# Arief-AK/OpenCL-Development-Real-time-Image-Processing

Measured on AMD Instinct MI355X. Metric: Mpixels/s (Gaussian 5x5, 4K RGBA), higher is better.
Workload: dtype u8 in/out, f32 accumulate

## Files before the change

### opencl-development-real-time-image-processing_amd/csrc/gauss_slide.hip

```cpp
#include <cmath>
#include <cstdlib>
#include <type_traits>

#include "common.hpp"
#include "kernels.hpp"
#include "slide_common.hpp"

namespace mi355 {

namespace {

constexpr uint32_t kRowStoreNowhere = 0x80000000u;
__device__ __forceinline__ void gstore_row_nt(global_ptr<uint8_t> rowp, uint32_t row_bytes, uint32_t off, u32x4 v)
{
    const auto rsrc = __builtin_amdgcn_make_buffer_rsrc((void*)rowp, (short)0, (int)row_bytes, 0x00020000);
    __builtin_amdgcn_raw_buffer_store_b128(v, rsrc, (int)off, 0, 2 );
}

constexpr uint32_t kSlideLdsForFiveWaves = 160u * 1024u / 5u - 1024u;
template <typename... KArgs, typename... Args>
hipError_t launch_slide_lds(void (*kernel)(KArgs...), const BandPlan& plan, uint32_t lds_bytes, hipStream_t stream,
                            Args... args)
{
    hipLaunchKernelGGL(kernel, dim3(plan.nblocks_a + plan.nblocks_b), dim3(kSlideWavesPerBlock * 64), lds_bytes, stream,
                       static_cast<KArgs>(args)...);
    return hipGetLastError();
}

template <int K>
struct Weights {
    float w[K];
};

__device__ __forceinline__ float ubyte_f32(uint32_t p, int c)
{
    return (float)((p >> (8 * c)) & 0xFFu);
}

__device__ __forceinline__ void cvt_pack4x4(const float (&h)[4][4] , u32x4& o)
{
    uint32_t o0, o1, o2, o3;
    asm("v_cvt_u32_f32_e32 %0, %4\n\t"
        "v_cvt_u32_f32_e32 %1, %5\n\t"
        "v_cvt_u32_f32_e32 %2, %6\n\t"
        "v_cvt_u32_f32_e32 %3, %7\n\t"
        "v_cvt_u32_f32_sdwa %0, %8 dst_sel:BYTE_1 dst_unused:UNUSED_PRESERVE src0_sel:DWORD\n\t"
        "v_cvt_u32_f32_sdwa %1, %9 dst_sel:BYTE_1 dst_unused:UNUSED_PRESERVE src0_sel:DWORD\n\t"
        "v_cvt_u32_f32_sdwa %2, %10 dst_sel:BYTE_1 dst_unused:UNUSED_PRESERVE src0_sel:DWORD\n\t"
        "v_cvt_u32_f32_sdwa %3, %11 dst_sel:BYTE_1 dst_unused:UNUSED_PRESERVE src0_sel:DWORD\n\t"
        "v_cvt_u32_f32_sdwa %0, %12 dst_sel:BYTE_2 dst_unused:UNUSED_PRESERVE src0_sel:DWORD\n\t"
        "v_cvt_u32_f32_sdwa %1, %13 dst_sel:BYTE_2 dst_unused:UNUSED_PRESERVE src0_sel:DWORD\n\t"
        "v_cvt_u32_f32_sdwa %2, %14 dst_sel:BYTE_2 dst_unused:UNUSED_PRESERVE src0_sel:DWORD\n\t"
        "v_cvt_u32_f32_sdwa %3, %15 dst_sel:BYTE_2 dst_unused:UNUSED_PRESERVE src0_sel:DWORD\n\t"
        "v_cvt_u32_f32_sdwa %0, %16 dst_sel:BYTE_3 dst_unused:UNUSED_PRESERVE src0_sel:DWORD\n\t"
        "v_cvt_u32_f32_sdwa %1, %17 dst_sel:BYTE_3 dst_unused:UNUSED_PRESERVE src0_sel:DWORD\n\t"
        "v_cvt_u32_f32_sdwa %2, %18 dst_sel:BYTE_3 dst_unused:UNUSED_PRESERVE src0_sel:DWORD\n\t"
        "v_cvt_u32_f32_sdwa %3, %19 dst_sel:BYTE_3 dst_unused:UNUSED_PRESERVE src0_sel:DWORD\n\t"
        "s_nop 1"
        : "=&v"(o0), "=&v"(o1), "=&v"(o2), "=&v"(o3)
        : "v"(h[0][0]), "v"(h[0][1]), "v"(h[0][2]), "v"(h[0][3]), "v"(h[1][0]), "v"(h[1][1]), "v"(h[1][2]),
          "v"(h[1][3]), "v"(h[2][0]), "v"(h[2][1]), "v"(h[2][2]), "v"(h[2][3]), "v"(h[3][0]), "v"(h[3][1]),
          "v"(h[3][2]), "v"(h[3][3]));
    o = u32x4{o0, o1, o2, o3};
}

__device__ __forceinline__ void cvt_pack3x4(const float (&h)[4][4] , uint32_t alpha_hi,
                                            u32x4& o)
{
    uint32_t o0, o1, o2, o3;
    asm("v_cvt_u32_f32_e32 %0, %4\n\t"
        "v_cvt_u32_f32_e32 %1, %5\n\t"
        "v_cvt_u32_f32_e32 %2, %6\n\t"
        "v_cvt_u32_f32_e32 %3, %7\n\t"
        "v_cvt_u32_f32_sdwa %0, %8 dst_sel:BYTE_1 dst_unused:UNUSED_PRESERVE src0_sel:DWORD\n\t"
        "v_cvt_u32_f32_sdwa %1, %9 dst_sel:BYTE_1 dst_unused:UNUSED_PRESERVE src0_sel:DWORD\n\t"
        "v_cvt_u32_f32_sdwa %2, %10 dst_sel:BYTE_1 dst_unused:UNUSED_PRESERVE src0_sel:DWORD\n\t"
        "v_cvt_u32_f32_sdwa %3, %11 dst_sel:BYTE_1 dst_unused:UNUSED_PRESERVE src0_sel:DWORD\n\t"
        "v_cvt_u32_f32_sdwa %0, %12 dst_sel:BYTE_2 dst_unused:UNUSED_PRESERVE src0_sel:DWORD\n\t"
        "v_cvt_u32_f32_sdwa %1, %13 dst_sel:BYTE_2 dst_unused:UNUSED_PRESERVE src0_sel:DWORD\n\t"
        "v_cvt_u32_f32_sdwa %2, %14 dst_sel:BYTE_2 dst_unused:UNUSED_PRESERVE src0_sel:DWORD\n\t"
        "v_cvt_u32_f32_sdwa %3, %15 dst_sel:BYTE_2 dst_unused:UNUSED_PRESERVE src0_sel:DWORD\n\t"
        "v_or_b32_e32 %0, %16, %0\n\t"
        "v_or_b32_e32 %1, %16, %1\n\t"
        "v_or_b32_e32 %2, %16, %2\n\t"
        "v_or_b32_e32 %3, %16, %3"
        : "=&v"(o0), "=&v"(o1), "=&v"(o2), "=&v"(o3)
        : "v"(h[0][0]), "v"(h[0][1]), "v"(h[0][2]), "v"(h[0][3]), "v"(h[1][0]), "v"(h[1][1]), "v"(h[1][2]),
          "v"(h[1][3]), "v"(h[2][0]), "v"(h[2][1]), "v"(h[2][2]), "v"(h[2][3]), "s"(alpha_hi));
    o = u32x4{o0, o1, o2, o3};
}

template <bool CLAMP>
__device__ __forceinline__ uint32_t to_u8(float a)
{
    if constexpr (CLAMP)
        a = fminf(a, 255.0f);
    return (uint32_t)a;
}

template <bool CLAMP>
__device__ __forceinline__ uint32_t pack_px(float a, float b, float c, float d)
{
    if constexpr (CLAMP) {
        a = fminf(a, 255.0f);
        b = fminf(b, 255.0f);
        c = fminf(c, 255.0f);
        d = fminf(d, 255.0f);
    }
    return (uint32_t)a | ((uint32_t)b << 8) | ((uint32_t)c << 16) | ((uint32_t)d << 24);
}

__device__ __forceinline__ void hpass5_dpp(float v0, float v1, float v2, float v3, float w0, float w1, float w2,
                                           float w3, float w4, float& o0, float& o1, float& o2, float& o3)
{
    asm volatile(
        "s_nop 1\n\t"
        "v_mul_f32_dpp %0, %6, %8 wave_shr:1 row_mask:0xf bank_mask:0xf bound_ctrl:1\n\t"
        "v_mul_f32_dpp %1, %7, %8 wave_shr:1 row_mask:0xf bank_mask:0xf bound_ctrl:1\n\t"
        "v_mul_f32_e32 %2, %8, %4\n\t"
        "v_mul_f32_e32 %3, %8, %5\n\t"
        "v_fmac_f32_dpp %0, %7, %9 wave_shr:1 row_mask:0xf bank_mask:0xf bound_ctrl:1\n\t"
        "v_fmac_f32_e32 %1, %9, %4\n\t"
        "v_fmac_f32_e32 %2, %9, %5\n\t"
        "v_fmac_f32_e32 %3, %9, %6\n\t"
        "v_fmac_f32_e32 %0, %10, %4\n\t"
        "v_fmac_f32_e32 %1, %10, %5\n\t"
        "v_fmac_f32_e32 %2, %10, %6\n\t"
        "v_fmac_f32_e32 %3, %10, %7\n\t"
        "v_fmac_f32_e32 %0, %11, %5\n\t"
        "v_fmac_f32_e32 %1, %11, %6\n\t"
        "v_fmac_f32_e32 %2, %11, %7\n\t"
        "v_fmac_f32_dpp %3, %4, %11 wave_shl:1 row_mask:0xf bank_mask:0xf bound_ctrl:1\n\t"
        "v_fmac_f32_e32 %0, %12, %6\n\t"
        "v_fmac_f32_e32 %1, %12, %7\n\t"
        "v_fmac_f32_dpp %2, %4, %12 wave_shl:1 row_mask:0xf bank_mask:0xf bound_ctrl:1\n\t"
        "v_fmac_f32_dpp %3, %5, %12 wave_shl:1 row_mask:0xf bank_mask:0xf bound_ctrl:1"
        : "=&v"(o0), "=&v"(o1), "=&v"(o2), "=&v"(o3)
        : "v"(v0), "v"(v1), "v"(v2), "v"(v3), "v"(w0), "v"(w1), "v"(w2), "v"(w3), "v"(w4));
}

struct SlideLane {
    global_ptr<const uint8_t> fin;
    global_ptr<uint8_t> fout;
    size_t row_bytes;
    SlideGeom g;
    int y0, nout, h;
    uint32_t px_off[4];
    int w;
    RaggedEdge edge;
};

template <bool NA0>
__device__ __forceinline__ bool alpha_row_differs(const u32x4& p, uint32_t nA)
{
    uint32_t t;
    if constexpr (NA0)
        t = (p.x & p.y) & (p.z & p.w);
    else
        t = ((p.x ^ nA) & (p.y ^ nA)) & ((p.z ^ nA) & (p.w ^ nA));
    return __builtin_amdgcn_ballot_w64(t < 0xFF000000u) != 0;
}

constexpr int kBandDone = 0;
constexpr int kBandAbortUniform = 1;
constexpr int kBandAbort = 2;
constexpr int kBandAbortUniformFirst = 3;

template <typename F, int... I>
__device__ __forceinline__ void static_rows_impl(F&& f, std::integer_sequence<int, I...>)
{
    (f(std::integral_constant<int, I>{}), ...);
}
template <int N, typename F>
__device__ __forceinline__ void static_rows(F&& f)
{
    static_rows_impl(f, std::make_integer_sequence<int, N>{});
}


template <int R, bool CLAMP, int NCH, bool RAGGED, bool UP, int AMODE, bool LOCKSTEP>
__device__ __forceinline__ int gauss_slide_band(const SlideLane& L, const float (&wv)[2 * R + 1], uint32_t alpha_hi,
                                                const uint32_t* __restrict__ alpha_tab, u32x4 (&q3)[2 * R + 1],
                                                bool preloaded)
{
    constexpr int K = 2 * R + 1;
    static_assert((NCH == 4) == (AMODE == 0), "AMODE 1 / 2 belong to the 3-channel pass");
    uint32_t in_off = L.g.in_off, out_off = L.g.out_off;
    [[maybe_unused]] const uint32_t out_voff = L.g.stores ? out_off : kRowStoreNowhere;
    const BandWalk W = band_walk(UP, L.y0, L.nout, R, L.h);
    uint32_t cur_nA = 0u;
    int run = 0;
    int code = kBandDone;
    const ptrdiff_t step_bytes = UP ? -(ptrdiff_t)L.row_bytes : (ptrdiff_t)L.row_bytes;
    const int y_lo = max(L.y0 - R, 0), y_hi = min(L.y0 + L.nout - 1 + R, L.h - 1);
    int y_in = W.y_first;
    auto in_p = L.fin + (size_t)clampi(y_in, y_lo, y_hi) * L.row_bytes;
    auto out_p = L.fout + (size_t)out_row(W, 0) * L.row_bytes;
    auto next_in_row = [&]() {
        const int y_next = y_in + W.y_step;
        in_p += (min(y_in, y_next) >= y_lo && max(y_in, y_next) <= y_hi) ? step_bytes : (ptrdiff_t)0;
        y_in = y_next;
    };
    auto load_row = [&]() -> u32x4 {
        const auto rowp = in_p;
        next_in_row();
        if constexpr (R <= 2)
            lane_offset_here(in_off);
        if constexpr (RAGGED) {
            if (L.w < 4) {
                u32x4 r;
#pragma unroll
                for (int j = 0; j < 4; j++)
                    r[j] = gload<uint32_t>(rowp + L.px_off[j]);
                return r;
            }
            return gload_a4<u32x4>(rowp + in_off);
        } else {
            return gload<u32x4>(rowp + in_off);
        }
    };

    constexpr int PF = (K < 3) ? K : 3;
    u32x4 q_own[K];
    u32x4 (&q)[K] = (AMODE == 0) ? q_own : q3;
    if (AMODE != 2 || !preloaded) {
#pragma unroll
        for (int u = 0; u < PF; u++)
            q[u] = load_row();
    } else {
#pragma unroll
        for (int u = 0; u < PF; u++)
            next_in_row();
    }
    if constexpr (AMODE == 1) {
        if (alpha_row_differs<true>(q[0], 0u)) {
            const uint32_t a_row = ((uint32_t)__builtin_amdgcn_readfirstlane((int)q[0].x) >> 24) & 0xFFu;
            return alpha_row_differs<false>(q[0], (a_row ^ 0xFFu) << 24) ? kBandAbort : kBandAbortUniformFirst;
        }
    }

    constexpr bool kRing = R <= 3;
    static_assert(kRing || !UP, "the accumulator form walks down only");
    float rows[K][4 * NCH] = {};

    auto do_row = [&](auto slot, auto outputs) __attribute__((always_inline)) {
        constexpr int u = decltype(slot)::value;
        constexpr bool OUT = decltype(outputs)::value;
        {
            u32x4 p_copy = q[u];
            u32x4& p = *((PF < K) ? &q[u] : &p_copy);
            if constexpr (LOCKSTEP) {
                __builtin_amdgcn_s_barrier();
            }
            if constexpr (PF < K)
                q[(u + PF) % K] = load_row();
            if (L.g.edge_strip) {
                if constexpr (!RAGGED) {
                    if (L.g.left_of_image)
                        p = u32x4{p.x, p.x, p.x, p.x};
                    if (L.g.right_of_image)
                        p = u32x4{p.w, p.w, p.w, p.w};
                } else if (L.w >= 4) {
                    if (L.g.left_of_image)
                        p = u32x4{p.x, p.x, p.x, p.x};
                    ragged_shift_clamp(p, L.edge);
                }
            }
            if constexpr (AMODE == 1) {
                if (alpha_row_differs<true>(p, 0u) && code == kBandDone) {
                    const uint32_t a_row = ((uint32_t)__builtin_amdgcn_readfirstlane((int)p.x) >> 24) & 0xFFu;
                    code = alpha_row_differs<false>(p, (a_row ^ 0xFFu) << 24) ? kBandAbort : kBandAbortUniform;
                }
            }
            if constexpr (AMODE == 2) {
                if (alpha_row_differs<false>(p, cur_nA)) {
                    const uint32_t a_new = ((uint32_t)__builtin_amdgcn_readfirstlane((int)p.x) >> 24) & 0xFFu;
                    const uint32_t nA = (a_new ^ 0xFFu) << 24;
                    if (alpha_row_differs<false>(p, nA))
                        code = kBandAbort;
                    cur_nA = nA;
                    alpha_hi = __builtin_amdgcn_readfirstlane(alpha_tab[a_new]);
                    run = 0;
                }
                run++;
            }
            if constexpr (kRing) {
#pragma unroll
                for (int px = 0; px < 4; px++)
#pragma unroll
                    for (int c = 0; c < NCH; c++)
                        rows[u][px * NCH + c] = ubyte_f32(p[px], c);
            } else {
#pragma unroll
                for (int px = 0; px < 4; px++) {
                    float f[NCH];
#pragma unroll
                    for (int c = 0; c < NCH; c++)
                        f[c] = ubyte_f32(p[px], c);
#pragma unroll
                    for (int j = 0; j < K; j++) {
                        const int sl = (u - j + K) % K;
#pragma unroll
                        for (int c = 0; c < NCH; c++)
                            rows[sl][px * NCH + c] =
                                (j == 0) ? wv[0] * f[c] : __builtin_fmaf(wv[j], f[c], rows[sl][px * NCH + c]);
                    }
                }
            }
            if constexpr (PF == K)
                q[u] = load_row();
            if constexpr (OUT) {
                if constexpr (AMODE == 2) {
                    if (run < K)
                        code = kBandAbort;
                }
                auto vsum = [&](int e) -> float {
                    if constexpr (!kRing)
                        return rows[(u + 1) % K][e];
                    float a = wv[0] * rows[UP ? u : (u + 1) % K][e];
#pragma unroll
                    for (int j = 1; j < K; j++)
                        a = __builtin_fmaf(wv[j], rows[UP ? (u - j + K) % K : (u + 1 + j) % K][e], a);
                    return a;
                };
                u32x4 o;
                if constexpr (R == 2) {
                    float hres[4][4];
#pragma unroll
                    for (int c = 0; c < NCH; c++)
                        hpass5_dpp(vsum(0 * NCH + c), vsum(1 * NCH + c), vsum(2 * NCH + c), vsum(3 * NCH + c), wv[0],
                                   wv[1], wv[2], wv[3], wv[4], hres[c][0], hres[c][1], hres[c][2], hres[c][3]);
                    if constexpr (CLAMP) {
#pragma unroll
                        for (int px = 0; px < 4; px++)
                            o[px] = (NCH == 4) ? pack_px<true>(hres[0][px], hres[1][px], hres[2][px], hres[3][px])
                                               : (pack_px<true>(hres[0][px], hres[1][px], hres[2][px], 0.0f) | alpha_hi);
                    } else if constexpr (NCH == 4) {
                        cvt_pack4x4(hres, o);
                    } else {
                        cvt_pack3x4(hres, alpha_hi, o);
                    }
                } else {
                    float v[4 * NCH];
#pragma unroll
                    for (int e = 0; e < 4 * NCH; e++)
                        v[e] = vsum(e);
#pragma unroll
                    for (int px = 0; px < 4; px++) {
                        float r4[4] = {0.0f, 0.0f, 0.0f, 0.0f};
#pragma unroll
                        for (int c = 0; c < NCH; c++) {
                            float sum = 0.0f;
#pragma unroll
                            for (int t = 0; t < K; t++) {
                                const int s = px - R + t;
                                float src;
                                if (s < 0)
                                    src = dpp_left(v[(4 + s) * NCH + c]);
                                else if (s > 3)
                                    src = dpp_right(v[(s - 4) * NCH + c]);
                                else
                                    src = v[s * NCH + c];
                                sum = (t == 0) ? wv[0] * src : __builtin_fmaf(wv[t], src, sum);
                            }
                            r4[c] = sum;
                        }
                        o[px] = pack_px<CLAMP>(r4[0], r4[1], r4[2], r4[3]);
                        if constexpr (NCH == 3)
                            o[px] |= alpha_hi;
                    }
                }
                const auto rowp = out_p;
                out_p += step_bytes;
                if constexpr (!RAGGED) {
                    gstore_row_nt(rowp, (uint32_t)L.row_bytes, out_voff, o);
                } else if (L.g.stores) {
                    if constexpr (R <= 2)
                        lane_offset_here(out_off);
                    if constexpr (RAGGED) {
                        if (L.g.edge_strip && L.g.x_lane + 3 >= L.w) {
#pragma unroll
                            for (int j = 0; j < 4; j++)
                                if (L.g.x_lane + j < L.w)
                                    gstore_a4<uint32_t>(rowp + out_off + 4 * j, o[j]);
                        } else {
                            gstore_a4<u32x4>(rowp + out_off, o);
                        }
                    } else {
                        gstore_nt<u32x4>(rowp + out_off, o);
                    }
                }
            }
        }
    };
    static_rows<2 * R>([&](auto v) __attribute__((always_inline)) { do_row(v, std::false_type{}); });
    const int ntrips = L.nout / K, rem = L.nout - ntrips * K;
    auto trip = [&]() __attribute__((always_inline)) {
        static_rows<K>([&](auto v) __attribute__((always_inline)) {
            do_row(std::integral_constant<int, (2 * R + decltype(v)::value) % K>{}, std::true_type{});
        });
    };
    constexpr int kPeeled = RAGGED ? 0 : 1;
    if (ntrips >= kPeeled) {
        if constexpr (kPeeled)
            trip();
        for (int t = kPeeled; t < ntrips && code == kBandDone; t++)
            trip();
    }
    auto rem_rows = [&](auto self, auto v) __attribute__((always_inline)) {
        constexpr int V = decltype(v)::value;
        if constexpr (V < K - 1) {
            if (V < rem) {
                do_row(std::integral_constant<int, (2 * R + V) % K>{}, std::true_type{});
                self(self, std::integral_constant<int, V + 1>{});
            }
        }
    };
    if (code == kBandDone)
        rem_rows(rem_rows, std::integral_constant<int, 0>{});
    return code;
}

template <int R, bool CLAMP, bool RAGGED, int MODE, bool LOCKSTEP>
__global__ __launch_bounds__(kSlideWavesPerBlock * 64, (R == 3 && MODE == 3) ? 3 : 1) void gauss_slide_kernel(
    const uint8_t* __restrict__ in, uint8_t* __restrict__ out, int w, int h, int nstrips, int lanes_out,
    BandPlan plan, Weights<2 * R + 1> wts, uint32_t alpha_hi, const uint32_t* __restrict__ alpha_tab,
    uint32_t* __restrict__ flags)
{
    constexpr int K = 2 * R + 1;
    const int lane = threadIdx.x & 63;
    SlideItem it;
    if (!slide_item(plan, nstrips, h, &it))
        return;
    if constexpr (MODE == 4) {
        if (flags[it.work] == 0)
            return;
    }
    SlideLane L;
    L.g = slide_geom<4>(it.strip, lanes_out, lane, w, 16u, 16u);
    L.y0 = it.y0;
    L.nout = it.nout;
    L.h = h;
    L.w = w;
    L.row_bytes = (size_t)w * 4;
    L.fin = uniform_ptr(in + it.frame * L.row_bytes * h);
    L.fout = uniform_ptr(out + it.frame * L.row_bytes * h);
    L.edge = RaggedEdge{false, false, false, false};
    if constexpr (RAGGED) {
        if (w >= 4)
            L.g.in_off = ragged_edge_setup(L.g.q_lane, L.g.q_load, w, &L.edge);
    }
#pragma unroll
    for (int j = 0; j < 4; j++)
        L.px_off[j] = (uint32_t)clampi(L.g.x_lane + j, 0, w - 1) * 4u;

    float wv[K];
#pragma unroll
    for (int j = 0; j < K; j++) {
        wv[j] = wts.w[j];
        asm volatile("" : "+v"(wv[j]));
    }

    const bool up = (it.band & 1) != 0;
    u32x4 q3[K];
    auto run = [&](auto amode, bool preloaded) -> int {
        constexpr int AMODE = decltype(amode)::value;
        constexpr int NCH = AMODE == 0 ? 4 : 3;
        if constexpr (R <= 3) {
            if (up)
                return gauss_slide_band<R, CLAMP, NCH, RAGGED, true, AMODE, LOCKSTEP>(L, wv, alpha_hi, alpha_tab, q3, preloaded);
        }
        return gauss_slide_band<R, CLAMP, NCH, RAGGED, false, AMODE, LOCKSTEP>(L, wv, alpha_hi, alpha_tab, q3, preloaded);
    };
    auto three_channels = [&]() -> int {
        int code = run(std::integral_constant<int, 1>{}, false);
        if (code == kBandAbortUniform || code == kBandAbortUniformFirst)
            code = run(std::integral_constant<int, 2>{}, code == kBandAbortUniformFirst);
        return code;
    };
    if constexpr (MODE == 0) {
        if (three_channels() != kBandDone)
            run(std::integral_constant<int, 0>{}, false);
    } else if constexpr (MODE == 3) {
        const int code = three_channels();
        if (lane == 0)
            flags[it.work] = code == kBandDone ? 0u : 1u;
    } else {
        run(std::integral_constant<int, 0>{}, false);
    }
}

template <int R>
bool slide_plan(int w, int h, int nframes, bool ragged, StripPlan* sp, BandPlan* plan)
{
    constexpr int K = 2 * R + 1;
    *sp = make_strip_plan(w);
    if (K == 5) {
        const bool big = (size_t)sp->nstrips * ((h + 23) / 24) * nframes >= 2800;
        const int rows = (big && !ragged) ? 15 : 24;
        return make_band_plan(h, sp->nstrips, nframes, 4, rows, rows, rows, 0.0, 12, plan);
    }
    return (K == 3)   ? make_band_plan(h, sp->nstrips, nframes, 5, 12, 12, 12, 0.0, 6, plan)
                      : make_band_plan(h, sp->nstrips, nframes, 3, 96, 270, 40, 0.1, 4 * R + 4, plan);
}

template <int R>
hipError_t launch_r(hipStream_t stream, const uint8_t* d_in, uint8_t* d_out, int w, int h, int nframes,
                    const GaussCoef& coef, uint32_t* d_flags)
{
    constexpr int K = 2 * R + 1;
    constexpr bool kSplit = R >= 3;
    StripPlan sp;
    BandPlan plan;
    const bool ragged = rows_ragged(w, d_in, 16, d_out, 16) || (size_t)w * 4 > kRowStoreNowhere;
    if (!slide_plan<R>(w, h, nframes, ragged, &sp, &plan) || (kSplit && !d_flags))
        return hipErrorInvalidValue;
    const int nstrips = sp.nstrips, lanes_out = sp.lanes_out;
    Weights<K> wts;
    for (int j = 0; j < K; j++)
        wts.w[j] = coef.h_w1d[j];
    double wsum = 0.0;
    for (int j = 0; j < K; j++)
        wsum += (double)coef.h_w1d[j];
    if (!coef.d_alpha_tab)
        return hipErrorInvalidValue;
    const uint32_t alpha_hi = coef.h_alpha_tab[255];
    const uint32_t* alpha_tab = coef.d_alpha_tab;
    const bool lockstep =
        R <= 2 && !ragged && nstrips % kSlideWavesPerBlock == 0 && plan.nwork_b == 0 && plan.nwork_a >= 8192u;
    const uint32_t lds_bytes = (R == 1 && !ragged) ? kSlideLdsForFiveWaves : 0u;
    auto launch = [&](auto kernel) {
        return launch_slide_lds(kernel, plan, lds_bytes, stream, d_in, d_out, w, h, nstrips, lanes_out, plan, wts, alpha_hi,
                                alpha_tab, d_flags);
    };
    return dispatch_bool(gauss_upper_clamp(wsum), [&](auto CL) {
        return dispatch_bool(ragged, [&](auto RG) {
            if constexpr (kSplit) {
                const hipError_t e = launch(gauss_slide_kernel<R, CL.value, RG.value, 3, false>);
                return e != hipSuccess ? e : launch(gauss_slide_kernel<R, CL.value, RG.value, 4, false>);
            } else if constexpr (RG.value) {
                return launch(gauss_slide_kernel<R, CL.value, true, 0, false>);
            } else {
                return dispatch_bool(
                    lockstep, [&](auto LS) { return launch(gauss_slide_kernel<R, CL.value, false, 0, LS.value>); });
            }
        });
    });
}

}

bool gauss_slide_supported(const uint8_t* d_in, const uint8_t* d_out, int w, int h, int k)
{
    (void)h;
    (void)w;
    if (k != 3 && k != 5 && k != 7 && k != 9)
        return false;
    return aligned_to(d_in, 4) && aligned_to(d_out, 4);
}

size_t gauss_slide_flag_items(int w, int h, int nframes, int k)
{
    StripPlan sp;
    BandPlan plan;
    const hipError_t e = dispatch_int(k, std::integer_sequence<int, 7, 9>{}, [&](auto K) {
        return slide_plan<K.value / 2>(w, h, nframes, false, &sp, &plan) ? hipSuccess : hipErrorInvalidValue;
    });
    return e == hipSuccess ? (size_t)plan.nwork_a + plan.nwork_b : 0;
}

hipError_t launch_gauss_slide(hipStream_t stream, const uint8_t* d_in, uint8_t* d_out, int w, int h,
                              int nframes, const GaussCoef& coef, uint32_t* d_flags)
{
    return dispatch_int(coef.k, std::integer_sequence<int, 3, 5, 7, 9>{}, [&](auto K) {
        return launch_r<K.value / 2>(stream, d_in, d_out, w, h, nframes, coef, d_flags);
    });
}

}
```

### opencl-development-real-time-image-processing_amd/csrc/slide_common.hpp

```cpp
#pragma once
#include <cstdint>
#include <cstdlib>

#include "common.hpp"

namespace mi355 {

constexpr int kSlideLanesOutMax = 62;
constexpr int kSlideWavesPerBlock = 4;

struct BandPlan {
    int rows_a, nbands_a, rows_b, nbands_b, y_split;
    uint32_t nwork_a, nwork_b, nblocks_a, nblocks_b;
};

struct StripPlan {
    int quads, nstrips, lanes_out;
};

inline StripPlan make_strip_plan(int w, int lanes_pref = 0)
{
    StripPlan s;
    s.quads = (w + 3) / 4;
    s.nstrips = (s.quads + kSlideLanesOutMax - 1) / kSlideLanesOutMax;
    s.lanes_out = (s.quads + s.nstrips - 1) / s.nstrips;
    if (lanes_pref > 0 && lanes_pref <= kSlideLanesOutMax && s.nstrips > 1) {
        s.lanes_out = lanes_pref;
        s.nstrips = (s.quads + lanes_pref - 1) / lanes_pref;
    }
    static const int tune_lanes = [] {
        const char* e = tune_env("MI355_TUNE_LANES_OUT");
        return e ? atoi(e) : 0;
    }();
    if (tune_lanes > 0 && tune_lanes <= kSlideLanesOutMax) {
        s.lanes_out = tune_lanes;
        s.nstrips = (s.quads + tune_lanes - 1) / tune_lanes;
    }
    return s;
}

inline bool make_band_plan(int h, int nstrips, int nframes, int waves_per_simd, int rows_min, int rows_max,
                           int rows_tail, double tail_frac, int rows_small, BandPlan* out)
{
    const double resident = 256.0 * 4.0 * waves_per_simd;
    double rows = (double)h * nstrips * nframes / (10.0 * resident);
    int rows_big = (int)(rows < rows_min ? rows_min : (rows > rows_max ? rows_max : rows));
    static const struct Tune {
        int band_rows = 0, tail_rows = 0;
        double tail_frac = -1.0;
        Tune()
        {
            if (const char* e = tune_env("MI355_TUNE_BAND_ROWS"))
                band_rows = atoi(e);
            if (const char* e = tune_env("MI355_TUNE_TAIL_ROWS"))
                tail_rows = atoi(e);
            if (const char* e = tune_env("MI355_TUNE_TAIL_FRAC"))
                tail_frac = atof(e);
        }
    } tune;
    while (rows_small > 0 && rows_big / 2 >= rows_small &&
           (size_t)nstrips * ((h + rows_big - 1) / rows_big) * nframes < 2800)
        rows_big /= 2;
    if (tune.band_rows > 0)
        rows_big = tune.band_rows;
    if (tune.tail_rows > 0)
        rows_tail = tune.tail_rows;
    if (tune.tail_frac >= 0.0)
        tail_frac = tune.tail_frac;
    BandPlan p{};
    int h_b = (int)(h * tail_frac);
    if (h_b < rows_tail || h - h_b < rows_big || tail_frac <= 0.0 || rows_tail >= rows_big)
        h_b = 0;
    const int h_a = h - h_b;
    p.nbands_a = (h_a + rows_big - 1) / rows_big;
    p.rows_a = (h_a + p.nbands_a - 1) / p.nbands_a;
    p.y_split = h_a;
    if (h_b > 0) {
        p.nbands_b = (h_b + rows_tail - 1) / rows_tail;
        p.rows_b = (h_b + p.nbands_b - 1) / p.nbands_b;
    } else {
        p.nbands_b = 0;
        p.rows_b = 1;
    }
    const size_t na = (size_t)nstrips * p.nbands_a * nframes, nb = (size_t)nstrips * p.nbands_b * nframes;
    if (na + nb > 0x3FFFFFFFull)
        return false;
    p.nwork_a = (uint32_t)na;
    p.nwork_b = (uint32_t)nb;
    p.nblocks_a = (p.nwork_a + kSlideWavesPerBlock - 1) / kSlideWavesPerBlock;
    p.nblocks_b = (p.nwork_b + kSlideWavesPerBlock - 1) / kSlideWavesPerBlock;
    *out = p;
    return true;
}

#ifdef __HIPCC__
template <typename... KArgs, typename... Args>
hipError_t launch_slide(void (*kernel)(KArgs...), const BandPlan& plan, hipStream_t stream, Args... args)
{
    hipLaunchKernelGGL(kernel, dim3(plan.nblocks_a + plan.nblocks_b), dim3(kSlideWavesPerBlock * 64), 0, stream,
                       static_cast<KArgs>(args)...);
    return hipGetLastError();
}

template <typename T>
using global_ptr = __attribute__((address_space(1))) T*;

template <typename T>
__device__ __forceinline__ global_ptr<T> uniform_ptr(T* p)
{
    const uint64_t v = reinterpret_cast<uint64_t>(p);
    const uint32_t lo = __builtin_amdgcn_readfirstlane((uint32_t)v);
    const uint32_t hi = __builtin_amdgcn_readfirstlane((uint32_t)(v >> 32));
    return (global_ptr<T>)(((uint64_t)hi << 32) | lo);
}

__device__ __forceinline__ void lane_offset_here(uint32_t& off)
{
    asm volatile("" : "+v"(off));
}

template <typename V>
__device__ __forceinline__ V gload(global_ptr<const uint8_t> p)
{
    return *(global_ptr<const V>)p;
}
template <typename V>
__device__ __forceinline__ V gload_a4(global_ptr<const uint8_t> p)
{
    typedef V __attribute__((aligned(4))) VA;
    return *(global_ptr<const VA>)p;
}
template <typename V>
__device__ __forceinline__ void gstore_nt(global_ptr<uint8_t> p, V v)
{
    __builtin_nontemporal_store(v, (global_ptr<V>)p);
}
template <typename V>
__device__ __forceinline__ void gstore_a4(global_ptr<uint8_t> p, V v)
{
    typedef V __attribute__((aligned(4))) VA;
    *(global_ptr<VA>)p = v;
}

template <typename V>
__device__ __forceinline__ void gstore_a1(global_ptr<uint8_t> p, V v)
{
    typedef V __attribute__((aligned(1))) VA;
    *(global_ptr<VA>)p = v;
}

struct RaggedEdge {
    bool sh1, sh2, sh3, sh4;
};

__device__ __forceinline__ uint32_t ragged_edge_setup(int q_lane, int q_load, int w, RaggedEdge* e)
{
    const int xs = min(4 * q_load, w - 4);
    const int shift = 4 * q_lane - xs;
    e->sh1 = shift >= 1;
    e->sh2 = shift >= 2;
    e->sh3 = shift >= 3;
    e->sh4 = shift >= 4;
    return (uint32_t)xs * 4u;
}

__device__ __forceinline__ void ragged_shift_clamp(u32x4& p, const RaggedEdge& e)
{
    p.x = e.sh3 ? p.w : (e.sh2 ? p.z : (e.sh1 ? p.y : p.x));
    p.y = e.sh2 ? p.w : (e.sh1 ? p.z : p.y);
    p.z = e.sh1 ? p.w : p.z;
}

struct SlideItem {
    int strip, band, y0, nout;
    uint32_t work;
    size_t frame;
};

__device__ __forceinline__ bool slide_item(const BandPlan& plan, int nstrips, int h, SlideItem* it)
{
    const bool tail = blockIdx.x >= plan.nblocks_a;
    const uint32_t blk = tail ? xcd_remap(blockIdx.x - plan.nblocks_a, plan.nblocks_b)
                              : xcd_remap(blockIdx.x, plan.nblocks_a);
    const uint32_t work =
        __builtin_amdgcn_readfirstlane(blk * kSlideWavesPerBlock + (uint32_t)(threadIdx.x >> 6));
    if (work >= (tail ? plan.nwork_b : plan.nwork_a))
        return false;
    const int nbands = tail ? plan.nbands_b : plan.nbands_a;
    const int band_rows = tail ? plan.rows_b : plan.rows_a;
    it->work = tail ? plan.nwork_a + work : work;
    it->strip = work % nstrips;
    const int band = (work / nstrips) % nbands;
    it->frame = work / ((uint32_t)nstrips * nbands);
    it->band = band;
    it->y0 = (tail ? plan.y_split : 0) + band * band_rows;
    it->nout = min(band_rows, (tail ? h : plan.y_split) - it->y0);
    return true;
}

struct SlideGeom {
    int q_lane, q_load, q_end, x_lane;
    bool left_of_image, right_of_image, edge_strip, stores;
    uint32_t in_off, out_off;
};

template <int PX, int HALO = 1, bool CAP_LOAD = true>
__device__ __forceinline__ SlideGeom slide_geom(int strip, int lanes_out, int lane, int w, uint32_t bytes_in,
                                                uint32_t bytes_out)
{
    static_assert(HALO == 1 || !CAP_LOAD, "the cap is written for one halo lane");
    const int quads = (w + PX - 1) >> (PX == 8 ? 3 : (PX == 4 ? 2 : 1));
    SlideGeom g;
    g.q_lane = strip * lanes_out + lane - HALO;
    g.q_load = clampi(g.q_lane, 0, CAP_LOAD ? min(quads - 1, (strip + 1) * lanes_out) : quads - 1);
    g.q_end = min((strip + 1) * lanes_out, quads);
    g.x_lane = PX * g.q_lane;
    g.left_of_image = g.q_lane < 0;
    g.right_of_image = g.q_lane >= quads;
    g.edge_strip = (strip == 0) || (PX * (strip * lanes_out + 64 - HALO) > w);
    g.stores = (lane >= HALO) && (g.q_lane < g.q_end);
    g.in_off = (uint32_t)g.q_load * bytes_in;
    g.out_off = (uint32_t)(g.stores ? g.q_lane : 0) * bytes_out;
    return g;
}

struct BandWalk {
    int y_first, y_step, halo, nin, h;
};

__device__ __forceinline__ BandWalk band_walk(bool up, int y0, int nout, int halo, int h)
{
    return BandWalk{up ? y0 + nout - 1 + halo : y0 - halo, up ? -1 : 1, halo, nout + 2 * halo, h};
}

template <Border B>
__device__ __forceinline__ int in_row(const BandWalk& b, int i)
{
    return border_index<B>(b.y_first + b.y_step * min(i, b.nin - 1), b.h);
}

__device__ __forceinline__ int out_row(const BandWalk& b, int m)
{
    return b.y_first + b.y_step * (m + b.halo);
}

template <int CTRL, bool ZERO>
__device__ __forceinline__ float dpp_move(float v, float edge)
{
    return __builtin_bit_cast(float, __builtin_amdgcn_update_dpp(__builtin_bit_cast(int, edge),
                                                                 __builtin_bit_cast(int, v), CTRL, 0xF, 0xF, ZERO));
}
__device__ __forceinline__ float dpp_left(float v) { return dpp_move<0x138, true>(v, 0.0f); }
__device__ __forceinline__ float dpp_right(float v) { return dpp_move<0x130, true>(v, 0.0f); }
__device__ __forceinline__ float dpp_left_or(float v, float edge) { return dpp_move<0x138, false>(v, edge); }
__device__ __forceinline__ float dpp_right_or(float v, float edge) { return dpp_move<0x130, false>(v, edge); }

__device__ __forceinline__ void edge_clamp_cols(u32x4& p, bool left_of_image, bool right_of_image)
{
    if (left_of_image)
        p = u32x4{p.x, p.x, p.x, p.x};
    if (right_of_image)
        p = u32x4{p.w, p.w, p.w, p.w};
}

__device__ __forceinline__ void edge_reflect_cols(u32x4& p, bool left_of_image, bool right_of_image)
{
    if (left_of_image)
        p.w = p.y;
    if (right_of_image)
        p.x = p.z;
}

template <Border B>
__device__ __forceinline__ void ragged_px_offsets(int x_lane, int w, uint32_t (&px_off)[4])
{
#pragma unroll
    for (int j = 0; j < 4; j++)
        px_off[j] = (uint32_t)border_index<B>(clampi(x_lane + j, -1, w), w) * 4u;
}

__device__ __forceinline__ u32x4 ragged_row_load(global_ptr<const uint8_t> rowp, const SlideGeom& g, int w,
                                                 uint32_t in_off, const uint32_t (&px_off)[4])
{
    u32x4 r;
    if (g.edge_strip && !(g.x_lane >= 0 && g.x_lane + 3 < w)) {
#pragma unroll
        for (int j = 0; j < 4; j++)
            r[j] = gload<uint32_t>(rowp + px_off[j]);
    } else {
        r = gload_a4<u32x4>(rowp + in_off);
    }
    return r;
}
#endif

}
```

Baseline: 768,100.

## Shrink K5/K3 bands, use bounded buffer loads, fast-div work decode, add stamps

Cuts the band height for large 5x5 workloads from 15 to 10 rows, and adds a 6-row option for 3x3, so more waves run in parallel. Input rows are now read with buffer loads whose record count drops to zero past the band's last row, so out-of-range reads return zero instead of overrunning. Work-item decoding swaps integer div/mod for precomputed multiply-shift division. It also moves the weight register pinning into the band function, pins kernel arguments to scalar registers, and adds optional clock-stamp instrumentation behind a tuning macro. Shorter bands re-read more halo rows, which adds input traffic per output row.

```diff
diff --git a/opencl-development-real-time-image-processing_amd/csrc/gauss_slide.hip b/opencl-development-real-time-image-processing_amd/csrc/gauss_slide.hip
--- a/opencl-development-real-time-image-processing_amd/csrc/gauss_slide.hip
+++ b/opencl-development-real-time-image-processing_amd/csrc/gauss_slide.hip
@@ -15,6 +15,13 @@
 {
     const auto rsrc = __builtin_amdgcn_make_buffer_rsrc((void*)rowp, (short)0, (int)row_bytes, 0x00020000);
     __builtin_amdgcn_raw_buffer_store_b128(v, rsrc, (int)off, 0, 2 );
+}
+
+constexpr bool kNoOverrun = true;
+__device__ __forceinline__ u32x4 gload_row(global_ptr<const uint8_t> rowp, uint32_t records, uint32_t off)
+{
+    const auto rsrc = __builtin_amdgcn_make_buffer_rsrc((void*)rowp, (short)0, (int)records, 0x00020000);
+    return __builtin_bit_cast(u32x4, __builtin_amdgcn_raw_buffer_load_b128(rsrc, (int)off, 0, 0));
 }
 
 constexpr uint32_t kSlideLdsForFiveWaves = 160u * 1024u / 5u - 1024u;
@@ -25,6 +32,28 @@
     hipLaunchKernelGGL(kernel, dim3(plan.nblocks_a + plan.nblocks_b), dim3(kSlideWavesPerBlock * 64), lds_bytes, stream,
                        static_cast<KArgs>(args)...);
     return hipGetLastError();
+}
+
+#ifdef MI355_TUNE_ENV
+constexpr uint32_t kStampSlots = 16384, kStampWords = 8, kStampEvery = 64;
+__device__ uint64_t* g_slide_stamps = nullptr;
+struct WaveStamps {
+    uint64_t t[4] = {0, 0, 0, 0}, wall0 = 0;
+    uint64_t* slot = nullptr;
+};
+#else
+struct WaveStamps {};
+#endif
+template <int I>
+__device__ __forceinline__ void stamp(WaveStamps& st, bool first_only = false)
+{
+#ifdef MI355_TUNE_ENV
+    if (st.slot && !(first_only && st.t[I] != 0))
+        st.t[I] = clock64();
+#else
+    (void)st;
+    (void)first_only;
+#endif
 }
 
 template <int K>
@@ -179,14 +208,13 @@
 
 
 template <int R, bool CLAMP, int NCH, bool RAGGED, bool UP, int AMODE, bool LOCKSTEP>
-__device__ __forceinline__ int gauss_slide_band(const SlideLane& L, const float (&wv)[2 * R + 1], uint32_t alpha_hi,
+__device__ __forceinline__ int gauss_slide_band(const SlideLane& L, const float (&ws)[2 * R + 1], uint32_t alpha_hi,
                                                 const uint32_t* __restrict__ alpha_tab, u32x4 (&q3)[2 * R + 1],
-                                                bool preloaded)
+                                                bool preloaded, WaveStamps& st)
 {
     constexpr int K = 2 * R + 1;
     static_assert((NCH == 4) == (AMODE == 0), "AMODE 1 / 2 belong to the 3-channel pass");
-    uint32_t in_off = L.g.in_off, out_off = L.g.out_off;
-    [[maybe_unused]] const uint32_t out_voff = L.g.stores ? out_off : kRowStoreNowhere;
+    uint32_t in_off = L.g.in_off;
     const BandWalk W = band_walk(UP, L.y0, L.nout, R, L.h);
     uint32_t cur_nA = 0u;
     int run = 0;
@@ -195,7 +223,7 @@
     const int y_lo = max(L.y0 - R, 0), y_hi = min(L.y0 + L.nout - 1 + R, L.h - 1);
     int y_in = W.y_first;
     auto in_p = L.fin + (size_t)clampi(y_in, y_lo, y_hi) * L.row_bytes;
-    auto out_p = L.fout + (size_t)out_row(W, 0) * L.row_bytes;
+    [[maybe_unused]] int rows_left = W.nin;
     auto next_in_row = [&]() {
         const int y_next = y_in + W.y_step;
         in_p += (min(y_in, y_next) >= y_lo && max(y_in, y_next) <= y_hi) ? step_bytes : (ptrdiff_t)0;
@@ -215,6 +243,10 @@
                 return r;
             }
             return gload_a4<u32x4>(rowp + in_off);
+        } else if constexpr (kNoOverrun) {
+            const uint32_t records = rows_left > 0 ? (uint32_t)L.row_bytes : 0u;
+            rows_left--;
+            return gload_row(rowp, records, in_off);
         } else {
             return gload<u32x4>(rowp + in_off);
         }
@@ -231,6 +263,16 @@
 #pragma unroll
         for (int u = 0; u < PF; u++)
             next_in_row();
+    }
+    stamp<1>(st, true);
+    uint32_t out_off = L.g.out_off;
+    [[maybe_unused]] const uint32_t out_voff = L.g.stores ? out_off : kRowStoreNowhere;
+    auto out_p = L.fout + (size_t)out_row(W, 0) * L.row_bytes;
+    float wv[K];
+#pragma unroll
+    for (int j = 0; j < K; j++) {
+        wv[j] = ws[j];
+        asm volatile("" : "+v"(wv[j]));
     }
     if constexpr (AMODE == 1) {
         if (alpha_row_differs<true>(q[0], 0u)) {
@@ -394,6 +436,7 @@
         }
     };
     static_rows<2 * R>([&](auto v) __attribute__((always_inline)) { do_row(v, std::false_type{}); });
+    stamp<2>(st, true);
     const int ntrips = L.nout / K, rem = L.nout - ntrips * K;
     auto trip = [&]() __attribute__((always_inline)) {
         static_rows<K>([&](auto v) __attribute__((always_inline)) {
@@ -429,6 +472,11 @@
 {
     constexpr int K = 2 * R + 1;
     const int lane = threadIdx.x & 63;
+    [[maybe_unused]] WaveStamps st;
+#ifdef MI355_TUNE_ENV
+    const uint64_t t_entry = clock64(), wall_entry = wall_clock64();
+#endif
+    slide_args_here(in, out, w, h, nstrips, lanes_out, alpha_hi, alpha_tab, flags);
     SlideItem it;
     if (!slide_item(plan, nstrips, h, &it))
         return;
@@ -436,6 +484,13 @@
         if (flags[it.work] == 0)
             return;
     }
+#ifdef MI355_TUNE_ENV
+    if (uint64_t* const base = g_slide_stamps; base && it.work % kStampEvery == 0) {
+        st.slot = base + (size_t)((it.work / kStampEvery) % kStampSlots) * kStampWords;
+        st.t[0] = t_entry;
+        st.wall0 = wall_entry;
+    }
+#endif
     SlideLane L;
     L.g = slide_geom<4>(it.strip, lanes_out, lane, w, 16u, 16u);
     L.y0 = it.y0;
@@ -454,13 +509,6 @@
     for (int j = 0; j < 4; j++)
         L.px_off[j] = (uint32_t)clampi(L.g.x_lane + j, 0, w - 1) * 4u;
 
-    float wv[K];
-#pragma unroll
-    for (int j = 0; j < K; j++) {
-        wv[j] = wts.w[j];
-        asm volatile("" : "+v"(wv[j]));
-    }
-
     const bool up = (it.band & 1) != 0;
     u32x4 q3[K];
     auto run = [&](auto amode, bool preloaded) -> int {
@@ -468,9 +516,9 @@
         constexpr int NCH = AMODE == 0 ? 4 : 3;
         if constexpr (R <= 3) {
             if (up)
-                return gauss_slide_band<R, CLAMP, NCH, RAGGED, true, AMODE, LOCKSTEP>(L, wv, alpha_hi, alpha_tab, q3, preloaded);
+                return gauss_slide_band<R, CLAMP, NCH, RAGGED, true, AMODE, LOCKSTEP>(L, wts.w, alpha_hi, alpha_tab, q3, preloaded, st);
         }
-        return gauss_slide_band<R, CLAMP, NCH, RAGGED, false, AMODE, LOCKSTEP>(L, wv, alpha_hi, alpha_tab, q3, preloaded);
+        return gauss_slide_band<R, CLAMP, NCH, RAGGED, false, AMODE, LOCKSTEP>(L, wts.w, alpha_hi, alpha_tab, q3, preloaded, st);
     };
     auto three_channels = [&]() -> int {
         int code = run(std::integral_constant<int, 1>{}, false);
@@ -488,7 +536,42 @@
     } else {
         run(std::integral_constant<int, 0>{}, false);
     }
-}
+#ifdef MI355_TUNE_ENV
+    if (st.slot) {
+        stamp<3>(st);
+        __builtin_amdgcn_s_waitcnt(0);
+        const uint64_t t_drained = clock64(), wall1 = wall_clock64();
+        if (lane == 0) {
+            st.slot[0] = st.t[0];
+            st.slot[1] = st.t[1];
+            st.slot[2] = st.t[2];
+            st.slot[3] = st.t[3];
+            st.slot[4] = t_drained;
+            st.slot[5] = st.wall0;
+            st.slot[6] = wall1;
+            st.slot[7] = ((uint64_t)it.nout << 32) | (it.work + 1u);
+        }
+    }
+#endif
+}
+
+#ifdef MI355_TUNE_ENV
+uint64_t* slide_stamps_buffer()
+{
+    static uint64_t* const d_buf = [] {
+        uint64_t* p = nullptr;
+        const size_t bytes = (size_t)kStampSlots * kStampWords * sizeof(uint64_t);
+        if (!tune_env("MI355_TUNE_STAMPS") || hipMalloc(&p, bytes) != hipSuccess)
+            return (uint64_t*)nullptr;
+        if (hipMemset(p, 0, bytes) != hipSuccess || hipMemcpyToSymbol(HIP_SYMBOL(g_slide_stamps), &p, sizeof(p)) != hipSuccess) {
+            (void)hipFree(p);
+            return (uint64_t*)nullptr;
+        }
+        return p;
+    }();
+    return d_buf;
+}
+#endif
 
 template <int R>
 bool slide_plan(int w, int h, int nframes, bool ragged, StripPlan* sp, BandPlan* plan)
@@ -497,11 +580,14 @@
     *sp = make_strip_plan(w);
     if (K == 5) {
         const bool big = (size_t)sp->nstrips * ((h + 23) / 24) * nframes >= 2800;
-        const int rows = (big && !ragged) ? 15 : 24;
+        const int rows = (big && !ragged) ? 10 : 24;
         return make_band_plan(h, sp->nstrips, nframes, 4, rows, rows, rows, 0.0, 12, plan);
     }
-    return (K == 3)   ? make_band_plan(h, sp->nstrips, nframes, 5, 12, 12, 12, 0.0, 6, plan)
-                      : make_band_plan(h, sp->nstrips, nframes, 3, 96, 270, 40, 0.1, 4 * R + 4, plan);
+    if (K == 3) {
+        const int rows = ((size_t)sp->nstrips * ((h + 11) / 12) * nframes >= 16384 && !ragged) ? 6 : 12;
+        return make_band_plan(h, sp->nstrips, nframes, 5, rows, rows, rows, 0.0, 6, plan);
+    }
+    return make_band_plan(h, sp->nstrips, nframes, 3, 96, 270, 40, 0.1, 4 * R + 4, plan);
 }
 
 template <int R>
@@ -516,6 +602,9 @@
     if (!slide_plan<R>(w, h, nframes, ragged, &sp, &plan) || (kSplit && !d_flags))
         return hipErrorInvalidValue;
     const int nstrips = sp.nstrips, lanes_out = sp.lanes_out;
+#ifdef MI355_TUNE_ENV
+    (void)slide_stamps_buffer();
+#endif
     Weights<K> wts;
     for (int j = 0; j < K; j++)
         wts.w[j] = coef.h_w1d[j];
@@ -550,6 +639,20 @@
 
 }
 
+#ifdef MI355_TUNE_ENV
+extern "C" __attribute__((visibility("default"))) int mi355_tune_slide_stamps(uint64_t* host_dst)
+{
+    uint64_t* const d_buf = slide_stamps_buffer();
+    if (!d_buf)
+        return 0;
+    const size_t bytes = (size_t)kStampSlots * kStampWords * sizeof(uint64_t);
+    if (hipDeviceSynchronize() != hipSuccess || hipMemcpy(host_dst, d_buf, bytes, hipMemcpyDeviceToHost) != hipSuccess ||
+        hipMemset(d_buf, 0, bytes) != hipSuccess)
+        return -1;
+    return (int)kStampSlots;
+}
+#endif
+
 bool gauss_slide_supported(const uint8_t* d_in, const uint8_t* d_out, int w, int h, int k)
 {
     (void)h;
diff --git a/opencl-development-real-time-image-processing_amd/csrc/slide_common.hpp b/opencl-development-real-time-image-processing_amd/csrc/slide_common.hpp
--- a/opencl-development-real-time-image-processing_amd/csrc/slide_common.hpp
+++ b/opencl-development-real-time-image-processing_amd/csrc/slide_common.hpp
@@ -9,10 +9,46 @@
 constexpr int kSlideLanesOutMax = 62;
 constexpr int kSlideWavesPerBlock = 4;
 
+#ifdef __HIPCC__
+#define MI355_HOST_DEVICE __host__ __device__
+#else
+#define MI355_HOST_DEVICE
+#endif
+
+struct FastDiv {
+    uint32_t mul, shift;
+};
+
+inline FastDiv make_fast_div(uint32_t d)
+{
+    uint32_t l = 0;
+    while ((1ull << l) < d)
+        l++;
+    return FastDiv{(uint32_t)(((1ull << (31 + l)) + d - 1) / d), l};
+}
+
+MI355_HOST_DEVICE inline uint32_t fast_div(uint32_t n, FastDiv f)
+{
+    return (uint32_t)(((uint64_t)(n << 1) * f.mul) >> 32) >> f.shift;
+}
+
 struct BandPlan {
     int rows_a, nbands_a, rows_b, nbands_b, y_split;
     uint32_t nwork_a, nwork_b, nblocks_a, nblocks_b;
-};
+    FastDiv by_strips, by_item_a, by_item_b;
+};
+
+struct SlideDecode {
+    uint32_t strip, band, frame;
+};
+
+MI355_HOST_DEVICE inline SlideDecode slide_decode(uint32_t work, uint32_t nstrips, uint32_t nbands, FastDiv by_strips,
+                                                  FastDiv by_item)
+{
+    const uint32_t t = fast_div(work, by_strips);
+    const uint32_t frame = fast_div(work, by_item);
+    return SlideDecode{work - t * nstrips, t - frame * nbands, frame};
+}
 
 struct StripPlan {
     int quads, nstrips, lanes_out;
@@ -89,6 +125,9 @@
     p.nwork_b = (uint32_t)nb;
     p.nblocks_a = (p.nwork_a + kSlideWavesPerBlock - 1) / kSlideWavesPerBlock;
     p.nblocks_b = (p.nwork_b + kSlideWavesPerBlock - 1) / kSlideWavesPerBlock;
+    p.by_strips = make_fast_div((uint32_t)nstrips);
+    p.by_item_a = make_fast_div((uint32_t)nstrips * (uint32_t)p.nbands_a);
+    p.by_item_b = make_fast_div((uint32_t)nstrips * (uint32_t)(p.nbands_b > 0 ? p.nbands_b : 1));
     *out = p;
     return true;
 }
@@ -177,8 +216,22 @@
     size_t frame;
 };
 
+__device__ __forceinline__ void slide_plan_here(const BandPlan& p)
+{
+    asm volatile("" ::"s"(p.rows_a), "s"(p.nbands_a), "s"(p.rows_b), "s"(p.nbands_b), "s"(p.y_split), "s"(p.nwork_a),
+                 "s"(p.nwork_b), "s"(p.nblocks_a), "s"(p.nblocks_b), "s"(p.by_strips.mul), "s"(p.by_strips.shift),
+                 "s"(p.by_item_a.mul), "s"(p.by_item_a.shift), "s"(p.by_item_b.mul), "s"(p.by_item_b.shift));
+}
+
+template <typename... T>
+__device__ __forceinline__ void slide_args_here(T... v)
+{
+    (([](auto x) __attribute__((always_inline)) { asm volatile("" ::"s"(x)); })(v), ...);
+}
+
 __device__ __forceinline__ bool slide_item(const BandPlan& plan, int nstrips, int h, SlideItem* it)
 {
+    slide_plan_here(plan);
     const bool tail = blockIdx.x >= plan.nblocks_a;
     const uint32_t blk = tail ? xcd_remap(blockIdx.x - plan.nblocks_a, plan.nblocks_b)
                               : xcd_remap(blockIdx.x, plan.nblocks_a);
@@ -189,9 +242,11 @@
     const int nbands = tail ? plan.nbands_b : plan.nbands_a;
     const int band_rows = tail ? plan.rows_b : plan.rows_a;
     it->work = tail ? plan.nwork_a + work : work;
-    it->strip = work % nstrips;
-    const int band = (work / nstrips) % nbands;
-    it->frame = work / ((uint32_t)nstrips * nbands);
+    const SlideDecode d =
+        slide_decode(work, (uint32_t)nstrips, (uint32_t)nbands, plan.by_strips, tail ? plan.by_item_b : plan.by_item_a);
+    it->strip = (int)d.strip;
+    it->frame = d.frame;
+    const int band = (int)d.band;
     it->band = band;
     it->y0 = (tail ? plan.y_split : 0) + band * band_rows;
     it->nout = min(band_rows, (tail ? h : plan.y_split) - it->y0);
```

Result: no change. 767,900, median of 2 (-0.0%).
